# huangzh13/StyleGAN.pytorch

Measured on AMD Instinct MI355X. Metric: img/s full G+D train step, 1024x1024 depth-9 bf16, higher is better.
Workload: dtype bf16; 1 GPU; ffhq1024: StyleGAN 1024x1024, progressive depth index 8, logistic+R1, alpha 0.5, batch 4/GPU, global batch 4; global_batch=4, parallelism=dp1

## Files before the change

### stylegan/pytorch_amd/GAN.py

```python
import contextlib
import copy
import datetime
import os
import random
import time
import timeit
from collections import OrderedDict

import numpy as np
import torch
import torch.nn as nn

from . import Losses
from . import functional as F
from .Blocks import DiscriminatorBlock, DiscriminatorTop, GSynthesisBlock, InputBlock
from .CustomLayers import EqualizedConv2d, EqualizedLinear, PixelNormLayer, Truncation, act_code, apply_act
from .data import get_data_loader
from . import native
from .native import ACT_LRELU
from .optim import FusedAdam, clip_and_step, ema_update


class DeferredLoss:

    __slots__ = ("_host", "_event", "_scale", "_value", "__weakref__")

    def __init__(self, dev_scalar, scale=1.0, stream=None):
        self._scale, self._value = float(scale), None
        if dev_scalar.is_cuda:
            with torch.cuda.stream(stream) if stream is not None else contextlib.nullcontext():
                t = dev_scalar.detach().reshape(1).float()
                view, slot = native.RING.take(4)
                self._host = view.view(torch.float32)
                self._host.copy_(t, non_blocking=True)
                self._event = native.RING.mark(slot, owner=self)
        else:
            self._host, self._event = dev_scalar.detach().reshape(1).float().clone(), None

    def item(self):
        if self._value is None:
            if self._event is not None:
                self._event.synchronize()
            self._value = float(self._host[0]) * self._scale
        return self._value

    __float__ = item

    def __format__(self, spec): return format(self.item(), spec)
    def __repr__(self): return repr(self.item())
    def __add__(self, o): return self.item() + float(o)
    __radd__ = __add__
    def __sub__(self, o): return self.item() - float(o)
    def __rsub__(self, o): return float(o) - self.item()
    def __mul__(self, o): return self.item() * float(o)
    __rmul__ = __mul__
    def __truediv__(self, o): return self.item() / float(o)
    def __lt__(self, o): return self.item() < float(o)
    def __gt__(self, o): return self.item() > float(o)
    def __eq__(self, o): return self.item() == float(o)
    def __abs__(self): return abs(self.item())
    def __neg__(self): return -self.item()
    def __hash__(self): return hash(self.item())


FUSE_RGB_FADE = os.environ.get("SGX_FUSE_RGB_FADE", "1") != "0"


def _nonlinearity(name):
    return {'relu': (nn.ReLU(), np.sqrt(2)), 'lrelu': (nn.LeakyReLU(negative_slope=0.2), np.sqrt(2))}[name]


def _conv_weights(module):
    ws = module.__dict__.get("_sgx_conv_weights")
    if ws is None:
        ws = [m.weight for m in module.modules() if isinstance(m, EqualizedConv2d)]
        module.__dict__["_sgx_conv_weights"] = ws
    return ws


def update_average(model_tgt, model_src, beta):
    ema_update(model_tgt, model_src, beta)


class GMapping(nn.Module):

    def __init__(self, latent_size=512, dlatent_size=512, dlatent_broadcast=None, mapping_layers=8, mapping_fmaps=512,
                 mapping_lrmul=0.01, mapping_nonlinearity='lrelu', use_wscale=True, normalize_latents=True, **kwargs):
        super().__init__()
        self.latent_size = latent_size
        self.mapping_fmaps = mapping_fmaps
        self.dlatent_size = dlatent_size
        self.dlatent_broadcast = dlatent_broadcast
        act, gain = _nonlinearity(mapping_nonlinearity)
        self._act = act_code(act)
        layers = []
        if normalize_latents:
            layers.append(('pixel_norm', PixelNormLayer()))
        layers.append(('dense0', EqualizedLinear(self.latent_size, self.mapping_fmaps, gain=gain, lrmul=mapping_lrmul,
                                                 use_wscale=use_wscale)))
        layers.append(('dense0_act', act))
        for layer_idx in range(1, mapping_layers):
            fmaps_in = self.mapping_fmaps
            fmaps_out = self.dlatent_size if layer_idx == mapping_layers - 1 else self.mapping_fmaps
            layers.append(('dense{:d}'.format(layer_idx),
                           EqualizedLinear(fmaps_in, fmaps_out, gain=gain, lrmul=mapping_lrmul, use_wscale=use_wscale)))
            layers.append(('dense{:d}_act'.format(layer_idx), act))
        self.map = nn.Sequential(OrderedDict(layers))
        self.mapping_layers = mapping_layers
        for m in self.map.modules():
            if isinstance(m, EqualizedLinear):
                m.first_order_only = True

    def forward(self, x):
        x = x.float()
        if hasattr(self.map, 'pixel_norm'):
            x = self.map.pixel_norm(x)
        for i in range(self.mapping_layers):
            dense = getattr(self.map, 'dense{:d}'.format(i))
# ... 495 lines not shown
        if st is None:
            st = self.__dict__["_aux_compute_stream"] = torch.cuda.Stream(device=self.device)
            quiet = getattr(torch.autograd.graph, "set_warn_on_accumulate_grad_stream_mismatch", None)
            if quiet is not None:
                quiet(False)
        return st

    def _param_stream(self, two_branches=False):
        if not self.param_stream:
            return torch.cuda.current_stream() if two_branches else None
        st = self.__dict__.get("_param_side_stream")
        if st is None:
            st = self.__dict__["_param_side_stream"] = torch.cuda.Stream(device=self.device)
        return st

    def _graphable(self, labels):
        return (self.use_graphs and labels is None and self.d_repeats == 1 and self.structure == "linear"
                and (self.dp is None or (self.gen.truncation is None
                                         and not isinstance(self.loss, Losses.RelativisticAverageHingeGAN))))

    def _d_grads(self, noise, real_batch, depth, alpha, labels=None):
        real_samples = self.progressive_down_sampling(real_batch, depth, alpha)

        def make_fakes():
            self._wait_update("g")
            with torch.no_grad():
                out = self.gen(noise, depth, alpha, labels)
            return out

        aux = self._aux_stream()
        lazy = isinstance(self.loss, Losses.LogisticGAN)
        self._wait_update("d")
        if aux is not None and lazy:
            self.dis.prepack(depth, (real_samples.shape[0], real_samples.shape[2], real_samples.shape[3], real_samples.shape[1]))
            cur = torch.cuda.current_stream()
            aux.wait_stream(cur)
            with torch.cuda.stream(aux):
                f_preds = self.dis(make_fakes(), depth, alpha)

            def fake_logits():
                cur.wait_stream(aux)
                f_preds.record_stream(cur)
                return f_preds
            loss = self.loss.dis_loss(real_samples, None, depth, alpha, fake_logits=fake_logits)
        elif self.conditional:
            loss = self.loss.dis_loss(real_samples, make_fakes(), labels, depth, alpha)
        else:
            loss = self.loss.dis_loss(real_samples, make_fakes if lazy else make_fakes(), depth, alpha)
        if self._ada_on():
            self.dis.ada_step()
        self._zero_grads("d", depth)
        side = self._param_stream(two_branches=aux is not None and lazy)
        self._sched_begin("d", depth, side)
        try:
            with F.accumulate_param_grads(), F.param_grad_stream(side):
                loss.backward()
        except BaseException:
            self._sched_abort()
            raise
        if side is not None:
            torch.cuda.current_stream().wait_stream(side)
        self._note_active_grads("d", depth)
        return loss.detach()

    def _reduce(self, kind):
        if self.dp is None:
            return
        sched = self.__dict__.pop("_sched_active", None)
        if sched is not None and not sched.recording and sched.gb is not None and sched.gb.attached():
            try:
                sched.finish()
            except RuntimeError:
                for key in [k for k, v in self.__dict__.get("_bucket_scheds", {}).items() if v is sched]:
                    self._bucket_scheds.pop(key, None)
                    self._grad_buckets.pop(key, None)
                raise
            self.__dict__["_last_sched"] = sched
            return
        gb = next((g for (k, _), g in self._grad_buckets.items() if k == kind and g.attached()), None)
        if gb is not None:
            self.dp.all_reduce_buckets(gb)
        else:
            self.dp.all_reduce_grads((self.dis if kind == "d" else self.gen).parameters())

    def _d_reduce(self):
        self._reduce("d")

    def _d_update(self):
        self.dis_optim.step()

    def _g_grads(self, noise, real_batch, depth, alpha, labels=None):
        real_samples = None
        if not isinstance(self.loss, (Losses.LogisticGAN, Losses.HingeGAN, Losses.StandardGAN, Losses.ConditionalGANLoss)):
            real_samples = self.progressive_down_sampling(real_batch, depth, alpha)
        self._wait_update("g")
        fake_samples = self.gen(noise, depth, alpha, labels)
        self._wait_update("d")
        d_all = self.__dict__.get("_sgx_dis_params")
        if d_all is None:
            d_all = self.__dict__["_sgx_dis_params"] = list(self.dis.parameters())
        d_params = [p for p in d_all if p.requires_grad]
        for p in d_params:
            p.requires_grad_(False)
        try:
            if self.conditional:
                loss = self.loss.gen_loss(real_samples, fake_samples, labels, depth, alpha)
            else:
                loss = self.loss.gen_loss(real_samples, fake_samples, depth, alpha)
            self._zero_grads("g", depth)
            side = self._param_stream()
            self._sched_begin("g", depth, side)
            try:
                with F.accumulate_param_grads(), F.param_grad_stream(side):
                    loss.backward()
            except BaseException:
                self._sched_abort()
                raise
            if side is not None:
                torch.cuda.current_stream().wait_stream(side)
            self._note_active_grads("g", depth)
        finally:
            for p in d_params:
                p.requires_grad_(True)
        return loss.detach()

    def _g_reduce(self):
        self._reduce("g")

    def _g_update(self):
        clip_and_step(self.gen_optim, max_norm=10.)
        if self.use_ema:
            self.ema_updater(self.gen_shadow, self.gen, self.ema_decay)

    def _async_update(self, kind, loss):
        upd = self.__dict__.get("_update_stream")
        if upd is None:
            upd = self.__dict__["_update_stream"] = torch.cuda.Stream(device=self.device)
        upd.wait_stream(torch.cuda.current_stream())
        with torch.cuda.stream(upd):
            (self._d_reduce if kind == "d" else self._g_reduce)()
            loss.record_stream(upd)
            loss = self.dp.all_reduce_scalar(loss)
            (self._d_update if kind == "d" else self._g_update)()
        ev = torch.cuda.Event()
        ev.record(upd)
        self.__dict__.setdefault("_pending_updates", {})[kind] = ev
        self.__dict__["_loss_stream"] = upd
        return loss

    def _wait_update(self, kind):
        ev = self.__dict__.get("_pending_updates", {}).pop(kind, None)
        if ev is not None:
            torch.cuda.current_stream().wait_event(ev)

    def _d_body(self, noise, real_batch, depth, alpha, labels=None):
        loss = self._d_grads(noise, real_batch, depth, alpha, labels)
        if self.dp is not None and not torch.cuda.is_current_stream_capturing():
            return self._async_update("d", loss)
        self._d_reduce()
        self._d_update()
        return loss

    def _g_body(self, noise, real_batch, depth, alpha, labels=None):
        loss = self._g_grads(noise, real_batch, depth, alpha, labels)
        if self.dp is not None and not torch.cuda.is_current_stream_capturing():
            return self._async_update("g", loss)
        self._g_reduce()
        self._g_update()
        return loss

    def _graphed(self, kind, noise, real_batch, depth, alpha):
        self._wait_update("d"); self._wait_update("g")
        key = (kind, int(depth), tuple(noise.shape), tuple(real_batch.shape), tuple(real_batch.stride()), real_batch.dtype,
               self.aux_stream, self.param_stream,
               self.dis._diffaug_bits, self.dis.training,
               None if self.dis.diffaug_override is None else self.dis.diffaug_override.data_ptr(),
               (self.dis.ada_target, self.dis.ada_interval, self.dis.ada_kimg) if self._ada_on() else None,
               None if not self._ada_on() or self.dis.ada_gate_override is None else self.dis.ada_gate_override.data_ptr())
        g = self._step_graphs.get(key)
        if g is None:
            g = self._step_graphs[key] = _StepGraph(self, kind, depth)
        return g.run(noise, real_batch, alpha)

    deferred_losses = False

    alpha_on_device = False

    def _alpha_arg(self, alpha):
        if not self.alpha_on_device or isinstance(alpha, torch.Tensor):
            return alpha
        return native.upload(torch.tensor([float(alpha), 1.0 - float(alpha)], dtype=torch.float32), self.device)[0]

    def _loss_out(self, deferred):
        return deferred if self.deferred_losses else deferred.item()

    def optimize_discriminator(self, noise, real_batch, depth, alpha, labels=None):
        if self._graphable(labels):
            return self._loss_out(self._graphed("d", noise, real_batch, depth, alpha))
        loss_val = None
        alpha = self._alpha_arg(alpha)
        for _ in range(self.d_repeats):
            loss = self._d_body(noise, real_batch, depth, alpha, labels)
            if loss_val is not None and self.__dict__.get("_loss_stream") is not None:
                torch.cuda.current_stream().wait_stream(self.__dict__.pop("_loss_stream"))
            loss_val = loss if loss_val is None else loss_val + loss
        return self._loss_out(DeferredLoss(loss_val, 1.0 / self.d_repeats, stream=self.__dict__.pop("_loss_stream", None)))

    def optimize_generator(self, noise, real_batch, depth, alpha, labels=None):
        if self._graphable(labels):
            return self._loss_out(self._graphed("g", noise, real_batch, depth, alpha))
        loss = self._g_body(noise, real_batch, depth, self._alpha_arg(alpha), labels)
        return self._loss_out(DeferredLoss(loss, stream=self.__dict__.pop("_loss_stream", None)))

    @staticmethod
    def fade_point_of(fade_in_percentage, epochs, total_batches):
        return int((fade_in_percentage / 100) * epochs * total_batches)

    @staticmethod
    def alpha_at(ticker, fade_point):
        return ticker / fade_point if ticker <= fade_point else 1

    @staticmethod
    def is_feedback_batch(i, total_batches, feedback_factor):
        return i % int(total_batches / feedback_factor + 1) == 0 or i == 1

    @staticmethod
    def is_checkpoint_epoch(epoch, epochs, checkpoint_factor):
# ... 322 lines not shown
```

### stylegan/pytorch_amd/csrc/rgbconv.hip

```cpp
#include "common.h"
#include <stdlib.h>

typedef __attribute__((ext_vector_type(4))) float f32x4_t;

typedef _Float16 h16x4 __attribute__((ext_vector_type(4)));
typedef _Float16 h16x2 __attribute__((ext_vector_type(2)));
typedef float f32x2 __attribute__((ext_vector_type(2)));
static __device__ __forceinline__ unsigned pack_f16x2(float lo, float hi) {
    const h16x2 v = {(_Float16)lo, (_Float16)hi};
    return __builtin_bit_cast(unsigned, v);
}
static __device__ __forceinline__ f32x4_t mma16h(s16x4 a, s16x4 b, f32x4_t c) {
    return __builtin_amdgcn_mfma_f32_16x16x16f16(__builtin_bit_cast(h16x4, a), __builtin_bit_cast(h16x4, b), c, 0, 0, 0);
}
static __device__ __forceinline__ f32x4_t mma16(s16x4 a, s16x4 b, f32x4_t c) {
    return __builtin_amdgcn_mfma_f32_16x16x16bf16_1k(a, b, c, 0, 0, 0);
}

__global__ void rgbconv_pack_kernel(const float* __restrict__ w0, float s0, const float* __restrict__ wr, float sr,
                                    const float* __restrict__ br, float bscale, bf16_t* __restrict__ wf, bf16_t* __restrict__ wd, int C) {
    const int tid = threadIdx.x + blockIdx.x * blockDim.x, nth = blockDim.x * gridDim.x;
    for (int e = tid; e < 3 * C * 16; e += nth) {
        const int ky = e / (C * 16), o = (e / 16) % C, k = e % 16, kx = k >> 2, j = k & 3;
        float v = 0.f;
// ... 471 lines not shown
                gzT[(v * 8 + 2 * q + 1) * TPS + p] = (bf16_t)(w[q] >> 16);
            }
        }
#pragma unroll
        for (int it = 0; it < NII; ++it) {
            const int idx = it * 256 + tid, rr = idx / (TW + 2), cr = idx - rr * (TW + 2);
            if (idx < NIP) {
                const unsigned p01 = pack_bf16x2(iv[it].r, iv[it].g), p23 = pack_bf16x2(iv[it].b, (((okm >> it) & 1u) && ones) ? 1.f : 0.f);
                const bf16_t vj[4] = {(bf16_t)(p01 & 0xffffu), (bf16_t)(p01 >> 16), (bf16_t)(p23 & 0xffffu), (bf16_t)(p23 >> 16)};
#pragma unroll
                for (int kx = 0; kx < 3; ++kx) {
                    const int c = cr - kx;
                    if (c >= 0 && c < TW) {
#pragma unroll
                        for (int j = 0; j < 4; ++j) imgT[(kx * 4 + j) * IPS + rr * TW + c] = vj[j];
                    }
                }
            }
        }
        __syncthreads();
        if (t + sc.stride < sc.end) load_tile(t + sc.stride);
        for (int g = wave; g < TH * 4; g += 4) {
            const int r = g >> 2, c0 = (g & 3) * 16 + 4 * l4;
            s16x4 af[CB];
#pragma unroll
            for (int cb = 0; cb < CB; ++cb) af[cb] = *reinterpret_cast<const s16x4*>(gzT + (cb * 16 + l15) * TPS + r * TW + c0);
#pragma unroll
            for (int ky = 0; ky < 3; ++ky) {
                const s16x4 bf = *reinterpret_cast<const s16x4*>(imgT + (nkx * 4 + nj) * IPS + (r + ky) * TW + c0);
#pragma unroll
                for (int cb = 0; cb < CB; ++cb) acc[cb][ky] = mma16(af[cb], bf, acc[cb][ky]);
            }
        }
        __syncthreads();
    }
    float* red = reinterpret_cast<float*>(smem);
#pragma unroll
    for (int cb = 0; cb < CB; ++cb)
#pragma unroll
        for (int ky = 0; ky < 3; ++ky)
#pragma unroll
            for (int rg = 0; rg < 4; ++rg) red[((wave * CB + cb) * 3 + ky) * 256 + rg * 64 + lane] = acc[cb][ky][rg];
    __syncthreads();
    for (int e = tid; e < CB * 3 * 256; e += 256) {
        const int cbky = e >> 8, rem = e & 255, rg = rem >> 6, ln = rem & 63, cb = cbky / 3, ky = cbky - cb * 3;
        float s = 0.f;
#pragma unroll
        for (int w = 0; w < 4; ++w) s += red[(w * CB * 3 + cbky) * 256 + rem];
        const int o = cb * 16 + 4 * (ln >> 4) + rg, n = ln & 15;
        part[(size_t)blockIdx.x * G::NOUT + (o * 3 + ky) * 16 + n] = s;
    }
}

__global__ __launch_bounds__(256) void rgbconv_wfinish_kernel(const float* __restrict__ part, float* __restrict__ out, int nblk, int nout) {
    __shared__ float red[256];
    const int tid = threadIdx.x, el = tid & 7, sl = tid >> 3, e = blockIdx.x * 8 + el;
    float s = 0.f;
    if (e < nout)
        for (int k = sl; k < nblk; k += 32) s += part[(size_t)k * nout + e];
    red[tid] = s;
    __syncthreads();
    if (tid < 8 && e < nout) {
        float tsum = 0.f;
        for (int k = 0; k < 32; ++k) tsum += red[k * 8 + tid];
        out[e] = tsum;
    }
}

__global__ __launch_bounds__(256) void rgbconv_chain_kernel(const float* __restrict__ dwp, const float* __restrict__ w0, float s0, const float* __restrict__ wr,
                                                            float sr, const float* __restrict__ br, float bscale, float* __restrict__ dw0, float* __restrict__ db0,
                                                            float* __restrict__ dwr, float* __restrict__ dbr, int acc, int C) {
    const int tid = threadIdx.x;
    if (dw0) {
        for (int e = tid; e < C * C * 9; e += 256) {
            const int o = e / (C * 9), i = (e / 9) % C, tap = e % 9, ky = tap / 3, kx = tap % 3;
            const float* d = dwp + (o * 3 + ky) * 16 + kx * 4;
            float v = s0 * sr * (d[0] * wr[i * 3] + d[1] * wr[i * 3 + 1] + d[2] * wr[i * 3 + 2]);
            if (br) v += s0 * d[3] * br[i] * bscale;
            dw0[e] = (acc & 1) ? dw0[e] + v : v;
        }
    }
    if (db0)
        for (int o = tid; o < C; o += 256) {
            const float v = dwp[(o * 3 + 1) * 16 + 4 + 3];
            db0[o] = (acc & 2) ? db0[o] + v : v;
        }
    for (int e = tid; e < C * 4; e += 256) {
        const int i = e >> 2, j = e & 3;
        float* dst = j < 3 ? (dwr ? dwr + i * 3 + j : nullptr) : (dbr ? dbr + i : nullptr);
        if (!dst) continue;
        float v = 0.f;
        for (int o = 0; o < C; ++o)
            for (int tap = 0; tap < 9; ++tap) v += dwp[(o * 3 + tap / 3) * 16 + (tap % 3) * 4 + j] * w0[(o * C + i) * 9 + tap];
        v *= j < 3 ? s0 * sr : s0 * bscale;
        const bool a = j < 3 ? (acc & 4) : (acc & 8);
        *dst = a ? *dst + v : v;
    }
}

static bool rgbconv_shape_ok(int B, int H, int W, int C, int dtype) {
    static const int on = [] { const char* e = getenv("SGX_RGBCONV"); return e ? atoi(e) : 1; }();
    return on && dtype == SGX_BF16 && (C == 16 || C == 32) && B >= 1 && H >= 16 && W >= 64 && H % 16 == 0 && W % 64 == 0;
}
extern "C" int sgx_rgbconv_ok(int B, int H, int W, int C, int dtype) { return rgbconv_shape_ok(B, H, W, C, dtype) ? 1 : 0; }

extern "C" int sgx_rgbconv_pack(const float* w0, float s0, const float* wr, float sr, const float* br, float bscale, void* wf, void* wd, int C,
                                void* stream) {
    SGX_REQUIRE(w0 && wr && wf && wd, SGX_EINVAL, "rgbconv_pack: null argument");
    SGX_REQUIRE(C == 16 || C == 32, SGX_EUNSUPPORTED, "rgbconv_pack: %d channels (16 or 32)", C);
    SGX_NOTE(0.0, 0.0, "rgbconv_pack C%d", C);
    hipLaunchKernelGGL(rgbconv_pack_kernel, dim3(C == 16 ? 12 : 24), dim3(256), 0, (hipStream_t)stream, w0, s0, wr, sr, br, bscale,
                       static_cast<bf16_t*>(wf), static_cast<bf16_t*>(wd), C);
    SGX_LAUNCH_CHECK("rgbconv_pack_kernel");
    return 0;
}

static int rc_ncu() { return sgx_ncu(); }
template <typename K>
static int rc_per_cu(K kern, int lds_bytes) {
    int n = 0;
    if (hipOccupancyMaxActiveBlocksPerMultiprocessor(&n, kern, 256, (size_t)lds_bytes) != hipSuccess || n < 1) n = 1;
    return n > 4 ? 4 : n;
}
static int rc_grid(int ntiles, int per_cu) {
    long g = (long)rc_ncu() * per_cu;
    if (g > ntiles) g = ntiles;
    g = (g + 7) / 8 * 8;
    return (int)g;
}

template <int CB, int EPI>
static int launch_rgbconv_fwd(const float* img, const bf16_t* wf, const float* b0, bf16_t* y, unsigned char* bits, int B, int H, int W, int ones,
                              hipStream_t st, bool one_shot = false) {
    using G = RcFwd<CB, EPI>;
    const int tiles_x = W / G::TW, tiles_y = H / G::TH, ntiles = B * tiles_x * tiles_y;
    sgx_lds_opt_in<rgbconv_fwd_kernel<CB, EPI>>(G::LDS);
    static const int per_cu = rc_per_cu(rgbconv_fwd_kernel<CB, EPI>, G::LDS);
    hipLaunchKernelGGL((rgbconv_fwd_kernel<CB, EPI>), dim3((unsigned)(one_shot ? (ntiles + 7) / 8 * 8 : rc_grid(ntiles, per_cu))), dim3(256), G::LDS, st, img, wf, b0, y, bits, B, H, W, ones,
                       tiles_x, tiles_y, ntiles);
    SGX_LAUNCH_CHECK("rgbconv_fwd_kernel");
    return 0;
}
struct RcTune { int fwd, nit, dbg; };
static RcTune& rc_tune() {
    static RcTune t = [] {
        RcTune r{RC_FWD_DEFAULT, 0, 0};
// ... 46 lines not shown
    }
    return C == 16 ? launch_rgbconv_fwd<1, 0>(img, w, b0, out, bt, B, H, W, ones, st) : launch_rgbconv_fwd<2, 0>(img, w, b0, out, bt, B, H, W, ones, st);
}

extern "C" int sgx_rgbconv_dgrad(const void* gz, const void* wd, float* gi, int B, int H, int W, int C, int dtype, void* stream) {
    SGX_REQUIRE(gz && wd && gi, SGX_EINVAL, "rgbconv_dgrad: null argument");
    SGX_REQUIRE(rgbconv_shape_ok(B, H, W, C, dtype), SGX_EUNSUPPORTED, "rgbconv_dgrad: shape B%d %dx%d C%d dtype %d (sgx_rgbconv_ok == 0)", B, H, W, C, dtype);
    const double px = (double)B * H * W;
    SGX_NOTE(2.0 * 27 * C * px, px * (12.0 + 2.0 * C), "rgbconv_dgrad B%d %dx%d %d->3", B, H, W, C);
    hipStream_t st = (hipStream_t)stream;
    const int nstrips = (W + RC_STRIP - 1) / RC_STRIP, nrb = (H + RC_ROWS - 1) / RC_ROWS;
    const unsigned grid = (unsigned)((((long)B * nstrips * nrb + 3) / 4 + 7) / 8 * 8);
    if (C == 16) hipLaunchKernelGGL((rgbconv_dgrad_kernel<1>), dim3(grid), dim3(256), 0, st, static_cast<const bf16_t*>(gz), static_cast<const bf16_t*>(wd), gi, B, H, W, nstrips, nrb);
    else hipLaunchKernelGGL((rgbconv_dgrad_kernel<2>), dim3(grid), dim3(256), 0, st, static_cast<const bf16_t*>(gz), static_cast<const bf16_t*>(wd), gi, B, H, W, nstrips, nrb);
    SGX_LAUNCH_CHECK("rgbconv_dgrad_kernel");
    return 0;
}

static int rgbconv_wgrad_blocks(int B, int H, int W) {
    const long ntiles = (long)B * (H / 8) * (W / 64);
    return rc_grid((int)(ntiles < (1 << 30) ? ntiles : (1 << 30)), 3);
}
extern "C" size_t sgx_rgbconv_wgrad_ws_bytes(int B, int H, int W, int C) {
    if (B < 1 || H < 8 || W < 64 || (C != 16 && C != 32)) return 0;
    return ((size_t)rgbconv_wgrad_blocks(B, H, W) + 1) * C * 48 * sizeof(float);
}
extern "C" int sgx_rgbconv_wgrad(const float* img, const void* gz, int ones, const float* w0, float s0, const float* wr, float sr, const float* br,
                                 float bscale, float* dw0, float* db0, float* dwr, float* dbr, int acc, void* ws, size_t ws_bytes, int B, int H, int W,
                                 int C, int dtype, void* stream) {
    SGX_REQUIRE(img && gz && w0 && wr && ws, SGX_EINVAL, "rgbconv_wgrad: null argument");
    SGX_REQUIRE(rgbconv_shape_ok(B, H, W, C, dtype), SGX_EUNSUPPORTED, "rgbconv_wgrad: shape B%d %dx%d C%d dtype %d (sgx_rgbconv_ok == 0)", B, H, W, C, dtype);
    SGX_REQUIRE(ws_bytes >= sgx_rgbconv_wgrad_ws_bytes(B, H, W, C), SGX_EWORKSPACE, "rgbconv_wgrad: workspace %zu < %zu", ws_bytes,
                sgx_rgbconv_wgrad_ws_bytes(B, H, W, C));
    SGX_REQUIRE(ones || (!db0 && !dbr), SGX_EINVAL, "rgbconv_wgrad: bias gradients need the bias channel (ones = 1)");
    hipStream_t st = (hipStream_t)stream;
    const int nblk = rgbconv_wgrad_blocks(B, H, W), nout = C * 48;
    const int tiles_x = W / 64, tiles_y = H / 8, ntiles = B * tiles_x * tiles_y;
    float* part = static_cast<float*>(ws);
    float* dwp = part + (size_t)nblk * nout;
    const double px = (double)B * H * W;
    SGX_NOTE(2.0 * 36 * C * px, px * (12.0 + 2.0 * C), "rgbconv_wgrad B%d %dx%d 3x%d", B, H, W, C);
    if (C == 16) {
        sgx_lds_opt_in<rgbconv_wgrad_kernel<1>>(RcWg<1>::LDS);
        hipLaunchKernelGGL((rgbconv_wgrad_kernel<1>), dim3((unsigned)nblk), dim3(256), RcWg<1>::LDS, st, img, static_cast<const bf16_t*>(gz), part, B, H, W,
                           ones, tiles_x, tiles_y, ntiles);
    } else {
        sgx_lds_opt_in<rgbconv_wgrad_kernel<2>>(RcWg<2>::LDS);
        hipLaunchKernelGGL((rgbconv_wgrad_kernel<2>), dim3((unsigned)nblk), dim3(256), RcWg<2>::LDS, st, img, static_cast<const bf16_t*>(gz), part, B, H, W,
                           ones, tiles_x, tiles_y, ntiles);
    }
    SGX_LAUNCH_CHECK("rgbconv_wgrad_kernel");
    hipLaunchKernelGGL(rgbconv_wfinish_kernel, dim3((unsigned)((nout + 7) / 8)), dim3(256), 0, st, (const float*)part, dwp, nblk, nout);
    SGX_LAUNCH_CHECK("rgbconv_wfinish_kernel");
    hipLaunchKernelGGL(rgbconv_chain_kernel, dim3(1), dim3(256), 0, st, (const float*)dwp, w0, s0, wr, sr, br, bscale, dw0, db0, dwr, dbr, acc, C);
    SGX_LAUNCH_CHECK("rgbconv_chain_kernel");
    return 0;
}
```

### stylegan/pytorch_amd/functional.py

```python
import contextlib
import functools
import os
import weakref

import numpy as np
import torch
from torch.autograd import Function
from torch.autograd.function import once_differentiable

from . import native as N

_DATA_GRAD_ONLY = 0


@contextlib.contextmanager
def data_grad_only():
    global _DATA_GRAD_ONLY
    _DATA_GRAD_ONLY += 1
    try:
        yield
    finally:
        _DATA_GRAD_ONLY -= 1


def _c(t):
    return t if t.is_contiguous() else t.contiguous()


class _NoGradCtx:
    needs_input_grad = (False,) * 16
    saved_tensors = ()

    def save_for_backward(self, *tensors):
        pass

    def mark_non_differentiable(self, *tensors):
        pass

    def set_materialize_grads(self, value):
        pass


def call(fn, *args):
    if torch.is_grad_enabled():
        for a in args:
            if isinstance(a, torch.Tensor) and a.requires_grad:
                return fn.apply(*args)
    return fn.forward(_NoGradCtx(), *args)


_bcall = call if os.environ.get("SGX_BWD_BYPASS", "1") != "0" else (lambda fn, *args: fn.apply(*args))


MODES = {"S": N.PACK_S, "D": N.PACK_D, "U": N.PACK_U, "UF": N.PACK_UF}
FWD_GEO = {"S": "S", "D": "D", "U": "U", "UF": "U"}
ADJ_GEO = {"S": "S", "D": "U", "U": "D", "UF": "D"}
_PACKS = {}
GRAD_NOTE = None
_WEIGHT_GEN = 0
_ACCUM_PARAM_GRADS = False
_PARAM_GRAD_STREAM = None


@contextlib.contextmanager
def param_grad_stream(stream):
    global _PARAM_GRAD_STREAM
    prev, _PARAM_GRAD_STREAM = _PARAM_GRAD_STREAM, stream
    try:
        yield
    finally:
        _PARAM_GRAD_STREAM = prev


_FAST_FORK = os.environ.get("SGX_FAST_FORK", "1") != "0"
_STREAMS = {}
# ... 570 lines not shown
        with torch.cuda.stream(side):
            launch()
        img.record_stream(side); gz.record_stream(side)
        for o in fresh:
            o.record_stream(cur)
    else:
        cur = _stream_of(cur_raw)
        N.check(N.lib().sgx_stream_wait_stream(side.cuda_stream, cur_raw), "sgx_stream_wait_stream")
        _set_stream(stream_id=side.stream_id, device_index=side.device_index, device_type=side.device_type)
        try:
            launch()
        finally:
            _set_stream(stream_id=cur.stream_id, device_index=cur.device_index, device_type=cur.device_type)
        img.record_stream(side); gz.record_stream(side)
        for o in fresh:
            o.record_stream(cur)
    if not accum:
        return tuple(outs)
    for p, w, o in zip(params, want, outs):
        if w:
            if p.grad is None:
                p.grad = o
            if GRAD_NOTE is not None:
                GRAD_NOTE(p)
    return None, None, None, None


class RgbConvBlurFn(Function):
    @staticmethod
    def forward(ctx, img, w0, b0, wr, br, s0, sr):
        img = _c(img)
        if img.dtype != torch.float32 or img.dim() != 4 or img.shape[3] != 3:
            raise N.SgxError("RgbConvBlurFn: fp32 NHWC RGB image expected")
        B, H, W, _ = img.shape
        C = w0.shape[0]
        wf, wd = rgb_packs(w0, s0, wr, sr, br)
        xb = torch.empty((B, H, W, C), dtype=torch.bfloat16, device=img.device)
        bits = torch.empty((B, H, W, C // 8), dtype=torch.uint8, device=img.device)
        N.check(N.lib().sgx_rgbconv_fwd(N.ptr(img), N.ptr(wf), N.ptr(None if b0 is None else _c(b0.detach())), N.ptr(xb), N.ptr(bits), B, H, W, C,
                                        1, 1, N.BF16, N.stream()), "sgx_rgbconv_fwd")
        ctx.cfg = (float(s0), float(sr))
        ctx.save_for_backward(img, w0, b0, wr, br)
        ctx.mark_non_differentiable(bits)
        ctx.set_materialize_grads(False)
        return xb, bits

    @staticmethod
    def backward(ctx, gz, _gbits=None):
        if gz is None:
            return (None,) * 7
        img, w0, b0, wr, br = ctx.saved_tensors
        s0, sr = ctx.cfg
        gz = _c(gz)
        gi = _bcall(RgbConvAdjFn, gz, w0, wr, br, s0, sr) if ctx.needs_input_grad[0] else None
        gw0 = gb0 = gwr = gbr = None
        if not _DATA_GRAD_ONLY:
            gw0, gb0, gwr, gbr = _bcall_wgrad(img, gz, True, w0, b0, wr, br, s0, sr, ctx.needs_input_grad[1:5])
        return gi, gw0, gb0, gwr, gbr, None, None


class RgbConvAdjFn(Function):
    @staticmethod
    def forward(ctx, gz, w0, wr, br, s0, sr):
        gz = _c(gz)
        B, H, W, C = gz.shape
        wf, wd = rgb_packs(w0, s0, wr, sr, br)
        gi = torch.empty((B, H, W, 3), dtype=torch.float32, device=gz.device)
        N.check(N.lib().sgx_rgbconv_dgrad(N.ptr(gz), N.ptr(wd), N.ptr(gi), B, H, W, C, N.dt(gz), N.stream()), "sgx_rgbconv_dgrad")
        ctx.cfg = (float(s0), float(sr))
        ctx.save_for_backward(gz, w0, wr, br)
        return gi

    @staticmethod
    def backward(ctx, gg):
        gz, w0, wr, br = ctx.saved_tensors
        s0, sr = ctx.cfg
        gg = _c(gg.float())
        ggz = _bcall(RgbConvPlainFn, gg, w0, wr, br, s0, sr) if ctx.needs_input_grad[0] else None
        gw0 = gwr = None
        if not _DATA_GRAD_ONLY:
            gw0, _, gwr, _ = _bcall_wgrad(gg, gz, False, w0, None, wr, br, s0, sr, (ctx.needs_input_grad[1], False, ctx.needs_input_grad[2], False))
        return ggz, gw0, gwr, None, None, None


class RgbConvPlainFn(Function):
    @staticmethod
    def forward(ctx, img, w0, wr, br, s0, sr):
        img = _c(img)
        B, H, W, _ = img.shape
        C = w0.shape[0]
        wf, wd = rgb_packs(w0, s0, wr, sr, br)
        z = torch.empty((B, H, W, C), dtype=torch.bfloat16, device=img.device)
        N.check(N.lib().sgx_rgbconv_fwd(N.ptr(img), N.ptr(wf), None, N.ptr(z), None, B, H, W, C, 0, 0, N.BF16, N.stream()), "sgx_rgbconv_fwd")
        ctx.cfg = (float(s0), float(sr))
        ctx.save_for_backward(img, w0, wr, br)
        return z

    @staticmethod
    def backward(ctx, gz):
        img, w0, wr, br = ctx.saved_tensors
        s0, sr = ctx.cfg
        gz = _c(gz)
        gi = _bcall(RgbConvAdjFn, gz, w0, wr, br, s0, sr) if ctx.needs_input_grad[0] else None
        gw0 = gwr = None
        if not _DATA_GRAD_ONLY:
            gw0, _, gwr, _ = _bcall_wgrad(img, gz, False, w0, None, wr, br, s0, sr, (ctx.needs_input_grad[1], False, ctx.needs_input_grad[2], False))
        return gi, gw0, gwr, None, None, None
# ... 166 lines not shown
        g, bits, wr, alpha_dev = ctx.saved_tensors
        ws, alpha, beta, need_img = ctx.cfg
        if ggy is None and ggp is None:
            return (None,) * 9
        dev = alpha_dev is not None
        L = N.lib()
        C = g.shape[-1]
        npix = g.numel() // C
        out = torch.empty_like(g)
        ggy_c = None if ggy is None else _c(ggy)
        ggp_c = None if ggp is None else _c(ggp)
        N.check(L.sgx_fade_rgb_bwd2(N.ptr(ggy_c), N.ptr(ggp_c), N.ptr(bits), N.ptr(_c(wr.detach())), ws * (1.0 if dev else beta), 0.0 if dev else alpha, 1.0,
                                    alpha_dev.data_ptr() if dev else None, N.ptr(out), npix, C, N.dt(g), N.stream()), "sgx_fade_rgb_bwd2")
        gwr = None
        if ggp_c is not None and ctx.needs_input_grad[3] and not _DATA_GRAD_ONLY:
            gwr = RgbWgradFn.forward(_NoGradCtx(), ggp_c, g, wr, ws * (1.0 if dev else beta))
            if dev:
                gwr = gwr * alpha_dev[1]
        return out, None, None, gwr, None, None, None, None, None


class ConvDownFadeRgbFn(Function):

    @staticmethod
    def forward(ctx, x, weight, bias, pimg, wr, br, scale, ipad, alpha, beta, ws, bs1, bs2, x_pre=None, x_pre_bits=None):
        x, pimg = _c(x), _c(pimg)
        fwd, adj = packs(weight, "D", scale, ipad, x.dtype)
        B, H, W, Cin = x.shape
        taps, Cout, K = fwd.shape
        if K != Cin or tuple(pimg.shape) != (B, H // 2, W // 2, 3) or pimg.dtype != torch.float32 or tuple(wr.shape) != (Cout, 3, 1, 1):
            raise N.SgxError("conv+fade(rgb): pooled fp32 image [B, H/2, W/2, 3] and a [Cout, 3, 1, 1] weight expected")
        y = torch.empty((B, H // 2, W // 2, Cout), dtype=x.dtype, device=x.device)
        bits = torch.empty((B, H // 2, W // 2, Cout // 8), dtype=torch.uint8, device=x.device)
        dev = isinstance(alpha, torch.Tensor)
        if dev and not (alpha.dtype == torch.float32 and alpha.numel() == 2 and alpha.is_contiguous()):
            raise N.SgxError("conv+fade(rgb): device coefficients must be a contiguous fp32 [alpha, beta] pair")
        N.check(N.lib().sgx_conv4x4s2_down_fade_rgb(N.ptr(x), N.ptr(fwd), N.ptr(None if bias is None else _c(bias.detach())), N.ptr(pimg),
                                                    N.ptr(_c(wr.detach())), float(ws), N.ptr(None if br is None else _c(br.detach())), float(bs1), float(bs2),
                                                    0.0 if dev else float(alpha), 0.0 if dev else float(beta), alpha.data_ptr() if dev else None,
                                                    N.ptr(y), N.ptr(bits), B, H, W, Cin, Cout, N.dt(x), N.stream()), "sgx_conv4x4s2_down_fade_rgb")
        ctx.cfg = ("D", scale, ipad, False, 0, bias is not None, False, False)
        ctx.bias_ref = weakref.ref(bias) if bias is not None else (lambda: None)
        ctx.br_ref = weakref.ref(br) if br is not None else (lambda: None)
        ctx.fade = ((None, None) if dev else (float(alpha), float(beta))) + (float(ws), float(bs1) * float(bs2))
        ctx.save_for_backward(x, weight, None, None, x_pre, x_pre_bits, bits, alpha if dev else None, pimg, wr)
        return y

    @staticmethod
    def backward(ctx, g):
        g = _c(g)
        bits, alpha_dev, pimg, wr = ctx.saved_tensors[6:10]
        alpha, beta, ws, bs = ctx.fade
        br = ctx.br_ref()
        need_img = ctx.needs_input_grad[3]
        want_w = ctx.needs_input_grad[4] and not _DATA_GRAD_ONLY
        want_b = br is not None and ctx.needs_input_grad[5] and not _DATA_GRAD_ONLY
        gpimg = gwr = gbr = None
        if torch.is_grad_enabled() and FUSE_FADE_BWD2 and not want_w and not want_b:
            gy, gpimg = FadeRgbBwdFn.apply(g, bits, pimg, wr, ws, alpha, beta, alpha_dev, bool(need_img))
        elif torch.is_grad_enabled():
            if alpha_dev is not None:
                g_res = _bcall(ScaleDevFn, g, alpha_dev[1:2])
                gy = _bcall(LReluBwdBitsFn, g, bits, 0.2, alpha_dev[0:1])
            else:
                g_res = g if beta == 1.0 else _bcall(ScaleFn, g, beta)
                gy = _bcall(LReluBwdBitsFn, g, bits, 0.2, alpha)
            if need_img:
                gpimg = _bcall(RgbOutFn, g_res, wr, None, ws)
            if want_w:
                gwr = _bcall(RgbWgradFn, pimg, g_res, wr, ws)
            if want_b:
                gbr = _bcall(ColSumFn, g_res, bs)
        else:
            L = N.lib()
            C = g.shape[-1]
            npix = g.numel() // C
            accum = _ACCUM_PARAM_GRADS and wr.is_leaf and (br is None or br.is_leaf)
            acc = 0
            dw = db = None
            if want_w and accum and wr.grad is not None:
                dw, acc = wr.grad, acc | 1
            if want_b and accum and br.grad is not None:
                db, acc = br.grad, acc | 2
            gy = torch.empty_like(g)
            if need_img:
                gpimg = torch.empty_like(pimg)
            wsb = L.sgx_fade_rgb_bwd_ws_bytes(npix, C)
            wsp = N.workspace(wsb, g.device)
            dev = alpha_dev is not None
            side = _PARAM_GRAD_STREAM if (accum and (want_w or want_b)) else None
            cur_raw = N.stream()
            if side is not None and side.cuda_stream == cur_raw:
                side = None
            if side is None:
                if want_w and dw is None:
                    dw = torch.empty(wr.shape, dtype=torch.float32, device=g.device)
                if want_b and db is None:
                    db = torch.empty(br.shape, dtype=torch.float32, device=g.device)
            N.check(L.sgx_fade_rgb_bwd(N.ptr(g), N.ptr(bits), N.ptr(pimg), N.ptr(_c(wr.detach())), ws, bs, 0.0 if dev else alpha, 0.0 if dev else beta,
                                       alpha_dev.data_ptr() if dev else None, N.ptr(gy), None if side is not None else N.ptr(dw),
                                       None if side is not None else N.ptr(db), acc, N.ptr(gpimg), N.ptr(wsp), wsb, npix, C,
                                       N.dt(g), cur_raw), "sgx_fade_rgb_bwd")
            if side is not None:
                fresh = []

                def finish():
                    nonlocal dw, db
# ... 317 lines not shown

POOL_FORK = os.environ.get("SGX_POOL_FORK", "1") != "0"


class PoolForkFn(Function):

    @staticmethod
    def forward(ctx, x, scale):
        y = Pool2Fn.forward(_NoGradCtx(), x, scale)
        ctx.scale = float(scale)
        ctx.set_materialize_grads(False)
        return x.view_as(x), y

    @staticmethod
    def backward(ctx, gx, gy):
        if gy is None:
            return gx, None
        if gx is None:
            return _bcall(Up2Fn, gy, ctx.scale), None
        return _bcall(UpAddFn, gx, gy, ctx.scale), None


def _dtype_code(dtype):
    return N.F32 if dtype == torch.float32 else N.BF16


def rgb_layout(weight):
    if weight.shape[1] == 3 and weight.shape[0] != 3:
        return 1, 3, weight.shape[0]
    if weight.shape[0] == 3:
        return weight.shape[1], 1, weight.shape[1]
    raise N.SgxError("1x1 convolution is built for the RGB layers (3 channels on one side)")


class RgbInFn(Function):

    @staticmethod
    def forward(ctx, img, weight, bias, wscale, out_dtype):
        img, w = _c(img), _c(weight.detach())
        sj, sc, C = rgb_layout(w)
        B, H, W, _ = img.shape
        y = torch.empty((B, H, W, C), dtype=out_dtype, device=img.device)
        N.check(N.lib().sgx_rgb_in(N.ptr(img), N.ptr(w), sj, sc, float(wscale), N.ptr(None if bias is None else _c(bias.detach())), N.ptr(y),
                                   B * H * W, C, _dtype_code(out_dtype), N.stream()), "sgx_rgb_in")
        ctx.has_bias, ctx.wscale = bias is not None, float(wscale)
        ctx.save_for_backward(img, weight)
        return y

    @staticmethod
    def backward(ctx, g):
        img, weight = ctx.saved_tensors
        g = _c(g)
        gi = gw = gb = None
        if ctx.needs_input_grad[0]:
            gi = _bcall(RgbOutFn, g, weight, None, ctx.wscale)
        if not _DATA_GRAD_ONLY:
            if ctx.needs_input_grad[1]:
                gw = _bcall(RgbWgradFn, img, g, weight, ctx.wscale)
            if ctx.has_bias and ctx.needs_input_grad[2]:
                gb = _bcall(ColSumFn, g, 1.0)
        return gi, gw, gb, None, None


class RgbOutFn(Function):

    @staticmethod
    def forward(ctx, x, weight, bias, wscale):
        x, w = _c(x), _c(weight.detach())
        sj, sc, C = rgb_layout(w)
        B, H, W, Cx = x.shape
        assert Cx == C
        img = torch.empty((B, H, W, 3), dtype=torch.float32, device=x.device)
        N.check(N.lib().sgx_rgb_out(N.ptr(x), N.ptr(w), sj, sc, float(wscale), N.ptr(None if bias is None else _c(bias.detach())), N.ptr(img),
                                    B * H * W, C, N.dt(x), N.stream()), "sgx_rgb_out")
        ctx.has_bias, ctx.wscale = bias is not None, float(wscale)
        ctx.save_for_backward(x, weight)
        return img

    @staticmethod
    def backward(ctx, g):
        x, weight = ctx.saved_tensors
        g = _c(g)
        gx = gw = gb = None
        if ctx.needs_input_grad[0]:
            gx = _bcall(RgbInFn, g, weight, None, ctx.wscale, x.dtype)
        if not _DATA_GRAD_ONLY:
            if ctx.needs_input_grad[1]:
                gw = _bcall(RgbWgradFn, g, x, weight, ctx.wscale)
            if ctx.has_bias and ctx.needs_input_grad[2]:
                gb = _bcall(ColSumFn, g, 1.0)
        return gx, gw, gb, None


RGB_FORK = os.environ.get("SGX_RGB_FORK", "1") != "0"


class RgbOutForkFn(Function):

    @staticmethod
    def forward(ctx, x, weight, bias, wscale):
        img = RgbOutFn.forward(ctx, x, weight, bias, wscale)
        ctx.set_materialize_grads(False)
        return x.view_as(x), img

    @staticmethod
    def backward(ctx, gx, g):
        if g is None:
# ... 671 lines not shown
```

Before: 295.9 img/s.

## Skip discriminator image-gradient kernels in D backward; parallelize rgbconv chain kernel

```diff
diff --git a/stylegan/pytorch_amd/GAN.py b/stylegan/pytorch_amd/GAN.py
--- a/stylegan/pytorch_amd/GAN.py
+++ b/stylegan/pytorch_amd/GAN.py
@@ -64,6 +64,10 @@
 
 
 FUSE_RGB_FADE = os.environ.get("SGX_FUSE_RGB_FADE", "1") != "0"
+
+
+def _d_real_image_grad():
+    return os.environ.get("SGX_D_REAL_IMAGE_GRAD", "0") not in ("0", "")
 
 
 def _nonlinearity(name):
@@ -665,9 +669,14 @@
         self._zero_grads("d", depth)
         side = self._param_stream(two_branches=aux is not None and lazy)
         self._sched_begin("d", depth, side)
+        image_grad = _d_real_image_grad()
+        image_alone = getattr(self.dis, "conditional", None) is False
         try:
-            with F.accumulate_param_grads(), F.param_grad_stream(side):
-                loss.backward()
+            with F.accumulate_param_grads(), F.param_grad_stream(side), F.no_image_grad(image_alone and not image_grad):
+                if image_grad:
+                    loss.backward()
+                else:
+                    loss.backward(inputs=self._d_trainable())
         except BaseException:
             self._sched_abort()
             raise
@@ -696,6 +705,15 @@
         else:
             self.dp.all_reduce_grads((self.dis if kind == "d" else self.gen).parameters())
 
+    def _dis_params(self):
+        d_all = self.__dict__.get("_sgx_dis_params")
+        if d_all is None:
+            d_all = self.__dict__["_sgx_dis_params"] = list(self.dis.parameters())
+        return d_all
+
+    def _d_trainable(self):
+        return [p for p in self._dis_params() if p.requires_grad]
+
     def _d_reduce(self):
         self._reduce("d")
 
@@ -709,10 +727,7 @@
         self._wait_update("g")
         fake_samples = self.gen(noise, depth, alpha, labels)
         self._wait_update("d")
-        d_all = self.__dict__.get("_sgx_dis_params")
-        if d_all is None:
-            d_all = self.__dict__["_sgx_dis_params"] = list(self.dis.parameters())
-        d_params = [p for p in d_all if p.requires_grad]
+        d_params = self._d_trainable()
         for p in d_params:
             p.requires_grad_(False)
         try:
@@ -786,6 +801,7 @@
         self._wait_update("d"); self._wait_update("g")
         key = (kind, int(depth), tuple(noise.shape), tuple(real_batch.shape), tuple(real_batch.stride()), real_batch.dtype,
                self.aux_stream, self.param_stream,
+               _d_real_image_grad(),
                self.dis._diffaug_bits, self.dis.training,
                None if self.dis.diffaug_override is None else self.dis.diffaug_override.data_ptr(),
                (self.dis.ada_target, self.dis.ada_interval, self.dis.ada_kimg) if self._ada_on() else None,
diff --git a/stylegan/pytorch_amd/csrc/rgbconv.hip b/stylegan/pytorch_amd/csrc/rgbconv.hip
--- a/stylegan/pytorch_amd/csrc/rgbconv.hip
+++ b/stylegan/pytorch_amd/csrc/rgbconv.hip
@@ -547,12 +547,22 @@
     }
 }
 
+constexpr int RC_WF_PF = 8;
 __global__ __launch_bounds__(256) void rgbconv_wfinish_kernel(const float* __restrict__ part, float* __restrict__ out, int nblk, int nout) {
     __shared__ float red[256];
     const int tid = threadIdx.x, el = tid & 7, sl = tid >> 3, e = blockIdx.x * 8 + el;
     float s = 0.f;
     if (e < nout)
-        for (int k = sl; k < nblk; k += 32) s += part[(size_t)k * nout + e];
+        for (int k0 = sl; k0 < nblk; k0 += 32 * RC_WF_PF) {
+            float v[RC_WF_PF];
+#pragma unroll
+            for (int u = 0; u < RC_WF_PF; ++u) {
+                const int k = k0 + 32 * u;
+                v[u] = part[(size_t)(k < nblk ? k : nblk - 1) * nout + e];
+            }
+#pragma unroll
+            for (int u = 0; u < RC_WF_PF; ++u) s = k0 + 32 * u < nblk ? s + v[u] : s;
+        }
     red[tid] = s;
     __syncthreads();
     if (tid < 8 && e < nout) {
@@ -562,31 +572,47 @@
     }
 }
 
+constexpr int RC_CHAIN_TERMS = 9 * 32;
+static int rgbconv_chain_blocks(int C) { return C + (C * C * 9 + 255) / 256; }
 __global__ __launch_bounds__(256) void rgbconv_chain_kernel(const float* __restrict__ dwp, const float* __restrict__ w0, float s0, const float* __restrict__ wr,
                                                             float sr, const float* __restrict__ br, float bscale, float* __restrict__ dw0, float* __restrict__ db0,
                                                             float* __restrict__ dwr, float* __restrict__ dbr, int acc, int C) {
+    __shared__ __attribute__((aligned(16))) float prod[4][RC_CHAIN_TERMS];
     const int tid = threadIdx.x;
-    if (dw0) {
-        for (int e = tid; e < C * C * 9; e += 256) {
+    if ((int)blockIdx.x >= C) {
+        const int blk = (int)blockIdx.x - C, e = blk * 256 + tid;
+        if (dw0 && e < C * C * 9) {
             const int o = e / (C * 9), i = (e / 9) % C, tap = e % 9, ky = tap / 3, kx = tap % 3;
             const float* d = dwp + (o * 3 + ky) * 16 + kx * 4;
             float v = s0 * sr * (d[0] * wr[i * 3] + d[1] * wr[i * 3 + 1] + d[2] * wr[i * 3 + 2]);
             if (br) v += s0 * d[3] * br[i] * bscale;
             dw0[e] = (acc & 1) ? dw0[e] + v : v;
         }
-    }
-    if (db0)
-        for (int o = tid; o < C; o += 256) {
-            const float v = dwp[(o * 3 + 1) * 16 + 4 + 3];
-            db0[o] = (acc & 2) ? db0[o] + v : v;
-        }
-    for (int e = tid; e < C * 4; e += 256) {
-        const int i = e >> 2, j = e & 3;
+        if (db0 && blk == 0 && tid < C) {
+            const float v = dwp[(tid * 3 + 1) * 16 + 4 + 3];
+            db0[tid] = (acc & 2) ? db0[tid] + v : v;
+        }
+        return;
+    }
+    if (!dwr && !dbr) return;
+    const int i = (int)blockIdx.x, nterm = 9 * C;
+    for (int t = tid; t < nterm; t += 256) {
+        const int o = t / 9, tap = t - o * 9;
+        const float4 d = *reinterpret_cast<const float4*>(dwp + (o * 3 + tap / 3) * 16 + (tap % 3) * 4);
+        const float w = w0[(o * C + i) * 9 + tap];
+        prod[0][t] = d.x * w; prod[1][t] = d.y * w; prod[2][t] = d.z * w; prod[3][t] = d.w * w;
+    }
+    __syncthreads();
+    if (tid < 4) {
+        const int j = tid;
         float* dst = j < 3 ? (dwr ? dwr + i * 3 + j : nullptr) : (dbr ? dbr + i : nullptr);
-        if (!dst) continue;
+        if (!dst) return;
         float v = 0.f;
-        for (int o = 0; o < C; ++o)
-            for (int tap = 0; tap < 9; ++tap) v += dwp[(o * 3 + tap / 3) * 16 + (tap % 3) * 4 + j] * w0[(o * C + i) * 9 + tap];
+#pragma unroll 6
+        for (int t = 0; t < nterm; t += 4) {
+            const float4 p = *reinterpret_cast<const float4*>(&prod[j][t]);
+            v += p.x; v += p.y; v += p.z; v += p.w;
+        }
         v *= j < 3 ? s0 * sr : s0 * bscale;
         const bool a = j < 3 ? (acc & 4) : (acc & 8);
         *dst = a ? *dst + v : v;
@@ -739,7 +765,7 @@
     SGX_LAUNCH_CHECK("rgbconv_wgrad_kernel");
     hipLaunchKernelGGL(rgbconv_wfinish_kernel, dim3((unsigned)((nout + 7) / 8)), dim3(256), 0, st, (const float*)part, dwp, nblk, nout);
     SGX_LAUNCH_CHECK("rgbconv_wfinish_kernel");
-    hipLaunchKernelGGL(rgbconv_chain_kernel, dim3(1), dim3(256), 0, st, (const float*)dwp, w0, s0, wr, sr, br, bscale, dw0, db0, dwr, dbr, acc, C);
+    hipLaunchKernelGGL(rgbconv_chain_kernel, dim3((unsigned)rgbconv_chain_blocks(C)), dim3(256), 0, st, (const float*)dwp, w0, s0, wr, sr, br, bscale, dw0, db0, dwr, dbr, acc, C);
     SGX_LAUNCH_CHECK("rgbconv_chain_kernel");
     return 0;
 }
diff --git a/stylegan/pytorch_amd/functional.py b/stylegan/pytorch_amd/functional.py
--- a/stylegan/pytorch_amd/functional.py
+++ b/stylegan/pytorch_amd/functional.py
@@ -21,6 +21,23 @@
         yield
     finally:
         _DATA_GRAD_ONLY -= 1
+
+
+_NO_IMAGE_GRAD = 0
+
+
+@contextlib.contextmanager
+def no_image_grad(on=True):
+    global _NO_IMAGE_GRAD
+    _NO_IMAGE_GRAD += 1 if on else 0
+    try:
+        yield
+    finally:
+        _NO_IMAGE_GRAD -= 1 if on else 0
+
+
+def _want_image_grad(ctx, k):
+    return ctx.needs_input_grad[k] and not (_NO_IMAGE_GRAD and not torch.is_grad_enabled())
 
 
 def _c(t):
@@ -697,7 +714,7 @@
         img, w0, b0, wr, br = ctx.saved_tensors
         s0, sr = ctx.cfg
         gz = _c(gz)
-        gi = _bcall(RgbConvAdjFn, gz, w0, wr, br, s0, sr) if ctx.needs_input_grad[0] else None
+        gi = _bcall(RgbConvAdjFn, gz, w0, wr, br, s0, sr) if _want_image_grad(ctx, 0) else None
         gw0 = gb0 = gwr = gbr = None
         if not _DATA_GRAD_ONLY:
             gw0, gb0, gwr, gbr = _bcall_wgrad(img, gz, True, w0, b0, wr, br, s0, sr, ctx.needs_input_grad[1:5])
@@ -970,7 +987,7 @@
         bits, alpha_dev, pimg, wr = ctx.saved_tensors[6:10]
         alpha, beta, ws, bs = ctx.fade
         br = ctx.br_ref()
-        need_img = ctx.needs_input_grad[3]
+        need_img = _want_image_grad(ctx, 3)
         want_w = ctx.needs_input_grad[4] and not _DATA_GRAD_ONLY
         want_b = br is not None and ctx.needs_input_grad[5] and not _DATA_GRAD_ONLY
         gpimg = gwr = gbr = None
@@ -1394,7 +1411,7 @@
         img, weight = ctx.saved_tensors
         g = _c(g)
         gi = gw = gb = None
-        if ctx.needs_input_grad[0]:
+        if _want_image_grad(ctx, 0):
             gi = _bcall(RgbOutFn, g, weight, None, ctx.wscale)
         if not _DATA_GRAD_ONLY:
             if ctx.needs_input_grad[1]:
```

Measured after the change: 299.4 img/s (median of 6 runs). +1.2%, better.
